# martinambrus/PitchExtractor

Measured on AMD Instinct MI355X. Metric: mel-frames/sec training throughput (JDCNet, 24 kHz, batch=256), higher is better.
Workload: dtype f32

## Files before the change

include/pitchextractor_hip.h:

```cpp
#ifndef PITCHEXTRACTOR_HIP_H
#define PITCHEXTRACTOR_HIP_H

#include <stddef.h>
#include <stdint.h>

#ifdef __cplusplus
extern "C" {
#endif

#define PE_OK 0
#define PE_E_ARG (-1)
#define PE_E_UNSUPPORTED (-2)
#define PE_E_WORKSPACE (-3)

enum pe_products {
  PE_PROD_NATIVE = 0,
  PE_PROD_X3 = 1,
  PE_PROD_H2 = 2,
  PE_PROD_BF16 = 3,
  PE_PROD_F16 = 4
};

int pe_abi_version(void);
int pe_device_count(void);
// ... 72 lines not shown
                         float eps, float momentum, float* running_mean, float* running_var, float* mean,
                         float* invstd, float* scale, float* shift, void* workspace, size_t workspace_bytes,
                         void* stream);
int pe_bn_eval_affine(const float* gamma, const float* beta, const float* running_mean,
                      const float* running_var, float eps, int C, float* scale, float* shift, void* stream);
int pe_bn_act_pool_fwd(int act16, const void* x, const float* scale, const float* shift, float slope, void* y, long rows,
                       int Fin, int C, int pool, long ldy, int coff, unsigned* amax_out, void* stream);
int pe_bn_act_pool_bwd(int act16, const void* x, const void* dy, const float* scale, const float* shift,
                       const float* mean, const float* invstd, float slope, void* dx, float* dgamma, float* dbeta,
                       long rows, int Fin, int C, int pool, long lddy, int coff, void* workspace,
                       size_t workspace_bytes, unsigned* amax_out, void* stream);
int pe_maxpool_fwd(int act16, const void* x, void* y, long rows, int Fin, int C, int pool, long ldy, int coff,
                   unsigned char* argmax_out, void* stream);
int pe_maxpool_bwd_add(int act16, const void* x, const unsigned char* argmax, const void* dy, void* dx, long rows,
                       int Fin, int C, int pool, long lddy, int coff, unsigned* amax_out, void* stream);
int pe_dropout_fwd(int act16, const void* x, long ldx, void* y, long ldy, const unsigned char* mask_in,
                   unsigned char* mask_out, long rows, int cols, float p, unsigned long long seed,
                   unsigned long long offset, void* stream);
int pe_nhwc_to_seq(int act16, const void* x, long ldx, int coff, float* seq, long rows, int C, void* stream);
int pe_seq_to_nhwc(int act16, const float* seq, void* x, long ldx, int coff, long rows, int C, int accumulate,
                   void* stream);
int pe_copy2d(int act16, const void* src, long lds, void* dst, long ldd, long rows, int cols, int accumulate,
              void* stream);

int pe_lstm_fwd(int ncells, const float* const* whh, float* const* gates, float* const* y,
                float* const* cbuf, const int* reverse, long ldy, int B, int T, int H, void* stream);
int pe_lstm_bwd(int ncells, const float* const* whh_t, float* const* gates, const float* const* cbuf,
                const float* const* dy, float* const* dcarry, const int* reverse, long lddy, int B, int T,
                int H, void* stream);
size_t pe_lstm_persistent_sync_bytes(int ncells, int B);
// ... 210 lines not shown
```

pitchextractor_amd/_lib.py:

```python
from __future__ import annotations

import ctypes as C
import os
from pathlib import Path

_PKG = Path(__file__).resolve().parent
LIB_PATH = Path(os.environ.get("PITCHEXTRACTOR_HIP_LIB", _PKG / "libpitchextractor_hip.so"))

_lib = None


class HipLibraryError(RuntimeError):
    pass


_p = C.c_void_p
_i = C.c_int
_l = C.c_long
_f = C.c_float
_d = C.c_double
_z = C.c_size_t
_u64 = C.c_ulonglong
_pp = C.POINTER(C.c_void_p)
_ip = C.POINTER(C.c_int)
# ... 28 lines not shown
    "pe_conv3x3_fwd_wf": (_i, [_i, _i, _p, _p, _p, _i, _i, _i, _i, _i, _i, _p, _p, _p, _p]),
    "pe_conv3x3_wgrad_workspace_bytes": (_z, [_i, _i, _i, _i, _i]),
    "pe_conv3x3_wgrad": (_i, [_i, _i, _p, _p, _p, _i, _i, _i, _i, _i, _p, _z, _p, _p, _p]),
    "pe_conv3x3_c1_stat_parts": (_i, [_i, _i, _i]),
    "pe_conv3x3_c1_fwd": (_i, [_i, _p, _l, _l, _l, _p, _p, _i, _i, _i, _p, _p]),
    "pe_conv3x3_c1_wgrad": (_i, [_i, _p, _l, _l, _l, _p, _p, _i, _i, _i, _p, _z, _p]),
    "pe_bn_workspace_bytes": (_z, [_i]),
    "pe_bn_train_stats": (_i, [_i, _p, _l, _i, _p, _p, _f, _f, _p, _p, _p, _p, _p, _p, _p, _z, _p]),
    "pe_conv3x3_wf_stat_parts": (_i, [_i, _i, _i]),
    "pe_bn_finalize_stats": (_i, [_p, _i, _l, _i, _p, _p, _f, _f, _p, _p, _p, _p, _p, _p, _p, _z, _p]),
    "pe_bn_eval_affine": (_i, [_p, _p, _p, _p, _f, _i, _p, _p, _p]),
    "pe_bn_act_pool_fwd": (_i, [_i, _p, _p, _p, _f, _p, _l, _i, _i, _i, _l, _i, _p, _p]),
    "pe_bn_act_pool_bwd": (_i, [_i, _p, _p, _p, _p, _p, _p, _f, _p, _p, _p, _l, _i, _i, _i, _l, _i, _p, _z, _p, _p]),
    "pe_maxpool_fwd": (_i, [_i, _p, _p, _l, _i, _i, _i, _l, _i, _p, _p]),
    "pe_maxpool_bwd_add": (_i, [_i, _p, _p, _p, _p, _l, _i, _i, _i, _l, _i, _p, _p]),
    "pe_dropout_fwd": (_i, [_i, _p, _l, _p, _l, _p, _p, _l, _i, _f, _u64, _u64, _p]),
    "pe_nhwc_to_seq": (_i, [_i, _p, _l, _i, _p, _l, _i, _p]),
    "pe_seq_to_nhwc": (_i, [_i, _p, _p, _l, _i, _l, _i, _i, _p]),
    "pe_copy2d": (_i, [_i, _p, _l, _p, _l, _l, _i, _i, _p]),
    "pe_lstm_fwd": (_i, [_i, _pp, _pp, _pp, _pp, _ip, _l, _i, _i, _i, _p]),
    "pe_lstm_bwd": (_i, [_i, _pp, _pp, _pp, _pp, _pp, _ip, _l, _i, _i, _i, _p]),
    "pe_lstm_persistent_sync_bytes": (_z, [_i, _i]),
    "pe_lstm_persistent_supported": (_i, [_i, _i, _i]),
    "pe_lstm_fwd_persistent": (_i, [_i, _i, _pp, _pp, _pp, _pp, _ip, _l, _i, _i, _i, _p, _p]),
    "pe_lstm_bwd_persistent_dbias_rows": (_i, [_i, _i, _i, _i, _l]),
    "pe_lstm_configure_stamps": (_i, [_i]),
    "pe_lstm_bwd_persistent": (_i, [_i, _i, _pp, _pp, _pp, _pp, _ip, _l, _i, _i, _i, _pp, _pp, _p, _p]),
    "pe_lstm_whh_grad_workspace_bytes": (_z, [_i, _i, _i]),
    "pe_lstm_whh_grad": (_i, [_i, _p, _p, _l, _p, _i, _i, _i, _i, _p, _z, _p, _p, _p]),
    "pe_colsum_workspace_bytes": (_z, [_i]),
# ... 140 lines not shown
```

pitchextractor_amd/csrc/elementwise.hip:

```cpp
#include <type_traits>
#include "forms.h"

namespace {
using namespace pe;

constexpr int kMaxPartials = 4096;

template <class F>
__device__ __forceinline__ void column_reduce2(F&& f, long n_pix, int C, double* partial ) {
  extern __shared__ __attribute__((aligned(16))) char smem_raw[];
  double* red = reinterpret_cast<double*>(smem_raw);
  const int quads = C >> 2;
  const int G = 256 / quads;
  const int q = threadIdx.x % quads, g = threadIdx.x / quads;
  double s1[4] = {0, 0, 0, 0}, s2[4] = {0, 0, 0, 0};
  if (g < G) {
    for (long p = (long)blockIdx.x * G + g; p < n_pix; p += (long)gridDim.x * G) {
      float4 a, b;
      f(p, q * 4, a, b);
      s1[0] += a.x; s1[1] += a.y; s1[2] += a.z; s1[3] += a.w;
      s2[0] += b.x; s2[1] += b.y; s2[2] += b.z; s2[3] += b.w;
    }
#pragma unroll
    for (int i = 0; i < 4; ++i) {
// ... 108 lines not shown
      const float4 v = ld4(xp + (long)j * C);
      float4 a;
      a.x = lrelu(fmaf(v.x, sc.x, sh.x), slope);
      a.y = lrelu(fmaf(v.y, sc.y, sh.y), slope);
      a.z = lrelu(fmaf(v.z, sc.z, sh.z), slope);
      a.w = lrelu(fmaf(v.w, sc.w, sh.w), slope);
      if (j == 0) m = a;
      else { m.x = fmaxf(m.x, a.x); m.y = fmaxf(m.y, a.y); m.z = fmaxf(m.z, a.z); m.w = fmaxf(m.w, a.w); }
    }
    st4(y + op * ldy + coff + q * 4, m);
    am = amax4(am, m);
  }
  amax_commit(am, amax);
}

__device__ __forceinline__ float dz_one(const float* __restrict__ xwin, long cstride, int j, int pool, float sc,
                                        float sh, float slope, float dyv) {
  float best = lrelu(fmaf(xwin[0], sc, sh), slope);
  int arg = 0;
  for (int k = 1; k < pool; ++k) {
    const float a = lrelu(fmaf(xwin[(long)k * cstride], sc, sh), slope);
    if (a > best) { best = a; arg = k; }
  }
  if (arg != j) return 0.f;
  const float z = fmaf(xwin[(long)j * cstride], sc, sh);
  return z > 0.f ? dyv : dyv * slope;
}

template <class TA>
struct BnBwdArgsT {
// ... 142 lines not shown
      [&](long item, int c, float4& s, float4& t) {
        BnWindow<POOL> w;
        bn_window<POOL, TA>(a, item, nwin, c, w, sc, sh);
        s = make_float4(0.f, 0.f, 0.f, 0.f);
        t = make_float4(0.f, 0.f, 0.f, 0.f);
#pragma unroll
        for (int j = 0; j < POOL; ++j) {
          s.x += w.dz[j].x; s.y += w.dz[j].y; s.z += w.dz[j].z; s.w += w.dz[j].w;
          t.x += w.dz[j].x * ((w.v[j].x - mu.x) * is.x); t.y += w.dz[j].y * ((w.v[j].y - mu.y) * is.y);
          t.z += w.dz[j].z * ((w.v[j].z - mu.z) * is.z); t.w += w.dz[j].w * ((w.v[j].w - mu.w) * is.w);
        }
      },
      n_items, a.C, partial);
}

template <int POOL, class TA>
__global__ __launch_bounds__(256) void bn_bwd_apply_win_kernel(const BnBwdArgsT<TA> a, long n_items, int nwin,
                                                               const float* __restrict__ c1,
                                                               const float* __restrict__ c2, TA* __restrict__ dx,
                                                               unsigned* __restrict__ amax) {
  const int quads = a.C >> 2;
  float am = 0.f;
  const int G = 256 / quads, c = (threadIdx.x % quads) * 4, g = threadIdx.x / quads;
  const float4 mu = *reinterpret_cast<const float4*>(a.mean + c), is = *reinterpret_cast<const float4*>(a.invstd + c);
  const float4 sc = *reinterpret_cast<const float4*>(a.scale + c), sh = *reinterpret_cast<const float4*>(a.shift + c);
  const float4 k1 = *reinterpret_cast<const float4*>(c1 + c), k2 = *reinterpret_cast<const float4*>(c2 + c);
  for (long item = (long)blockIdx.x * G + g; g < G && item < n_items; item += (long)gridDim.x * G) {
    BnWindow<POOL> w;
    bn_window<POOL, TA>(a, item, nwin, c, w, sc, sh);
#pragma unroll
    for (int j = 0; j < POOL; ++j) {
      if (j >= w.n) break;
      float4 o;
      o.x = sc.x * (w.dz[j].x - k1.x - (w.v[j].x - mu.x) * is.x * k2.x);
      o.y = sc.y * (w.dz[j].y - k1.y - (w.v[j].y - mu.y) * is.y * k2.y);
      o.z = sc.z * (w.dz[j].z - k1.z - (w.v[j].z - mu.z) * is.z * k2.z);
      o.w = sc.w * (w.dz[j].w - k1.w - (w.v[j].w - mu.w) * is.w * k2.w);
      st4(dx + (w.p0 + j) * a.C + c, o);
      am = amax4(am, o);
    }
  }
  amax_commit(am, amax);
}

template <class TA>
__global__ __launch_bounds__(256) void maxpool_fwd_kernel(const TA* __restrict__ x, TA* __restrict__ y,
                                                          long n_out_pix, int Fin, int C, int pool, long ldy,
                                                          int coff, unsigned char* __restrict__ arg) {
  const int quads = C >> 2, Fout = Fin / pool;
  const long total = n_out_pix * quads;
  for (long i = (long)blockIdx.x * 256 + threadIdx.x; i < total; i += (long)gridDim.x * 256) {
    const int q = (int)(i % quads);
    const long op = i / quads, row = op / Fout;
    const int fo = (int)(op % Fout);
// ... 298 lines not shown

extern "C" int pe_bn_act_pool_fwd(int act16, const void* x, const float* scale, const float* shift, float slope, void* y,
                                  long rows, int Fin, int C, int pool, long ldy, int coff, unsigned* amax_out,
                                  void* stream) {
  return with_act(act16, [&](auto a) {
    using TA = typename decltype(a)::TA;
    return bn_act_pool_fwd_impl(static_cast<const TA*>(x), scale, shift, slope, static_cast<TA*>(y), rows, Fin, C, pool,
                                ldy, coff, amax_out, stream);
  });
}

template <class TA>
static int bn_act_pool_bwd_impl(const TA* x, const TA* dy, const float* scale, const float* shift, const float* mean,
                                const float* invstd, float slope, TA* dx, float* dgamma, float* dbeta, long rows,
                                int Fin, int C, int pool, long lddy, int coff, void* workspace, size_t workspace_bytes,
                                unsigned* amax_out, void* stream) {
  if (!x || !dy || !scale || !shift || !mean || !invstd || !dx || !dgamma || !dbeta || rows <= 0) return PE_E_ARG;
  if (!bn_channels_ok(C) || (lddy & 3) || (coff & 3) || pool <= 0) return PE_E_UNSUPPORTED;
  const size_t need = pe_bn_workspace_bytes(C) + 2 * (size_t)C * sizeof(float);
  if (!workspace || workspace_bytes < need) return PE_E_WORKSPACE;
  hipStream_t st = pe_stream(stream);
  BnBwdArgsT<TA> a{x, dy, scale, shift, mean, invstd, slope, rows * Fin, Fin, C, pool, lddy, coff};
  double* partial = reinterpret_cast<double*>(workspace);
  float* c1 = reinterpret_cast<float*>(reinterpret_cast<char*>(workspace) + pe_bn_workspace_bytes(C));
  float* c2 = c1 + C;
  const int nwin = Fin / pool + (Fin % pool ? 1 : 0);
  const long n_items = rows * nwin;
  const bool win = pool == 1 || pool == 2 || pool == 4;
  if (!win && !std::is_same<TA, float>::value) return PE_E_UNSUPPORTED;
  const int grid = reduce_grid(win ? n_items : a.n_in_pix, C,
                               (!std::is_same<TA, float>::value && pool == 1) ? kMaxPartials : 1024);
  if (pool == 1)
    hipLaunchKernelGGL((bn_bwd_partial_win_kernel<1, TA>), dim3(grid), dim3(256), reduce_lds(C), st, a, n_items, nwin, partial);
  else if (pool == 2)
    hipLaunchKernelGGL((bn_bwd_partial_win_kernel<2, TA>), dim3(grid), dim3(256), reduce_lds(C), st, a, n_items, nwin, partial);
  else if (pool == 4)
    hipLaunchKernelGGL((bn_bwd_partial_win_kernel<4, TA>), dim3(grid), dim3(256), reduce_lds(C), st, a, n_items, nwin, partial);
  else if constexpr (std::is_same<TA, float>::value)
    hipLaunchKernelGGL(bn_bwd_partial_kernel, dim3(grid), dim3(256), reduce_lds(C), st, a, partial);
  PE_LAUNCH_CHECK();
  hipLaunchKernelGGL(bn_bwd_finalize_kernel, dim3(pe_cdiv(C, 4)), dim3(256), 0, st, partial, grid, a.n_in_pix, C,
                     dgamma, dbeta, c1, c2);
  PE_LAUNCH_CHECK();
  const int agrid = win ? ew_grid(pe_cdiv(n_items, 256 / (C / 4)) * 256L) : ew_grid(a.n_in_pix * (C / 4));
  if (pool == 1)
    hipLaunchKernelGGL((bn_bwd_apply_win_kernel<1, TA>), dim3(agrid), dim3(256), 0, st, a, n_items, nwin, c1, c2, dx,
                       amax_out);
  else if (pool == 2)
    hipLaunchKernelGGL((bn_bwd_apply_win_kernel<2, TA>), dim3(agrid), dim3(256), 0, st, a, n_items, nwin, c1, c2, dx,
                       amax_out);
  else if (pool == 4)
    hipLaunchKernelGGL((bn_bwd_apply_win_kernel<4, TA>), dim3(agrid), dim3(256), 0, st, a, n_items, nwin, c1, c2, dx,
                       amax_out);
  else if constexpr (std::is_same<TA, float>::value)
    hipLaunchKernelGGL(bn_bwd_apply_kernel, dim3(agrid), dim3(256), 0, st, a, c1, c2, dx, amax_out);
  PE_LAUNCH_CHECK();
  return PE_OK;
}

extern "C" int pe_bn_act_pool_bwd(int act16, const void* x, const void* dy, const float* scale, const float* shift,
                                  const float* mean, const float* invstd, float slope, void* dx, float* dgamma,
                                  float* dbeta, long rows, int Fin, int C, int pool, long lddy, int coff,
                                  void* workspace, size_t workspace_bytes, unsigned* amax_out, void* stream) {
  return with_act(act16, [&](auto a) {
    using TA = typename decltype(a)::TA;
    return bn_act_pool_bwd_impl(static_cast<const TA*>(x), static_cast<const TA*>(dy), scale, shift, mean, invstd, slope,
                                static_cast<TA*>(dx), dgamma, dbeta, rows, Fin, C, pool, lddy, coff, workspace,
                                workspace_bytes, amax_out, stream);
  });
}

template <class TA>
static int maxpool_fwd_impl(const TA* x, TA* y, long rows, int Fin, int C, int pool, long ldy, int coff,
                            unsigned char* argmax_out, void* stream) {
  if (!x || !y || rows <= 0 || Fin <= 0 || pool <= 0) return PE_E_ARG;
  if ((C & 3) || (ldy & 3) || (coff & 3) || (argmax_out && pool > 255)) return PE_E_UNSUPPORTED;
  const long n_out = rows * (Fin / pool);
  hipLaunchKernelGGL(maxpool_fwd_kernel<TA>, dim3(ew_grid(n_out * (C / 4))), dim3(256), 0, pe_stream(stream), x, y,
                     n_out, Fin, C, pool, ldy, coff, argmax_out);
  PE_LAUNCH_CHECK();
  return PE_OK;
}

extern "C" int pe_maxpool_fwd(int act16, const void* x, void* y, long rows, int Fin, int C, int pool, long ldy, int coff,
                              unsigned char* argmax_out, void* stream) {
  return with_act(act16, [&](auto a) {
// ... 124 lines not shown
```

pitchextractor_amd/model.py:

```python
from __future__ import annotations

import math
import os

import torch
from torch import nn

from . import ops

_ALIGN = 4


class _Conv(nn.Module):

    def __init__(self, cin, cout, k):
        super().__init__()
        self.weight = nn.Parameter(torch.empty(cout, cin, k, k))


class _BatchNorm(nn.Module):
    def __init__(self, c, eps=1e-5, momentum=0.1):
        super().__init__()
        self.eps, self.momentum = eps, momentum
        self.weight = nn.Parameter(torch.ones(c))
# ... 137 lines not shown
        st = ops.bn_train_stats(x, mod.weight, mod.bias, mod.running_mean, mod.running_var, mod.eps, mod.momentum,
                                partials=partials)
        mod.num_batches_tracked += 1
        return st
    return ops.bn_eval_affine(mod.weight, mod.bias, mod.running_mean, mod.running_var, mod.eps)


def _flat2(t):
    return t.view(-1, t.shape[-1])


def _no_amax(_param):
    return None


def _res_forward(blk: _ResBlock, x, pool, train, need_grad, slope, x_stats=None, wa=_no_amax):
    s = _Ctx()
    s.x = x
    s.bn_pre = _bn(blk.pre_conv[0], x, train, x_stats)
    s.am_p = ops.amax_word()
    s.p = ops.bn_act_pool_fwd(x, s.bn_pre, pool=pool, slope=slope, amax_out=s.am_p)
    out = ops.gemm_nt(_flat2(s.p), blk.conv1by1.weight.view(blk.cout, blk.cin), amax_a=s.am_p,
                      amax_b=wa(blk.conv1by1.weight))
    out = out.view(*s.p.shape[:3], blk.cout)
    wf0, s.wd0 = ops.conv3x3_repack(blk.conv[0].weight, True, need_grad, amax=wa(blk.conv[0].weight))
    s.c, c_stats = ops.conv3x3_fwd(s.p, wf0, bn_stats=train, amax=s.am_p)
    s.bn_mid = _bn(blk.conv[1], s.c, train, c_stats)
    s.am_a = ops.amax_word()
    s.a = ops.bn_act_pool_fwd(s.c, s.bn_mid, pool=1, slope=slope, amax_out=s.am_a)
    wf3, s.wd3 = ops.conv3x3_repack(blk.conv[3].weight, True, need_grad, amax=wa(blk.conv[3].weight))
    _, out_stats = ops.conv3x3_fwd(s.a, wf3, out=out, accumulate=True, bn_stats=train,
                                   amax=s.am_a)
    return out, s, out_stats


def _res_backward(blk: _ResBlock, s, d_out, pool, slope, grads, side, am_do=None, wa=_no_amax):
    if am_do is None:
        am_do = ops.amax_for(d_out)
    side.run(lambda: (ops.conv3x3_wgrad(s.a, d_out, grads[blk.conv[3].weight], amax_x=s.am_a, amax_dy=am_do),
                      ops.gemm_tn(_flat2(d_out), _flat2(s.p), out=grads[blk.conv1by1.weight].view(blk.cout, blk.cin),
                                  amax_a=am_do, amax_b=s.am_p)),
             d_out, am_do, on=OVERLAP_CONV_WGRAD)
    with ops.timer_tag("dgrad"):
        d_a = ops.conv3x3_fwd(d_out, s.wd3, amax=am_do)
    am_dc = ops.amax_word()
    d_c = ops.bn_act_pool_bwd(s.c, d_a, s.bn_mid, grads[blk.conv[1].weight], grads[blk.conv[1].bias], pool=1,
                              slope=slope, dx=d_a, amax_out=am_dc)
    side.run(lambda: ops.conv3x3_wgrad(s.p, d_c, grads[blk.conv[0].weight], amax_x=s.am_p, amax_dy=am_dc), d_c, am_dc,
             on=OVERLAP_CONV_WGRAD)
    with ops.timer_tag("dgrad"):
        d_p = ops.conv3x3_fwd(d_c, s.wd0, amax=am_dc)
    w1t = ops.transpose2d(blk.conv1by1.weight.view(blk.cout, blk.cin))
    ops.gemm_nt(_flat2(d_out), w1t, out=_flat2(d_p), accumulate=True, amax_a=am_do, amax_b=wa(blk.conv1by1.weight))
    am_dx = ops.amax_word()
    return ops.bn_act_pool_bwd(s.x, d_p, s.bn_pre, grads[blk.pre_conv[0].weight], grads[blk.pre_conv[0].bias],
                               pool=pool, slope=slope, amax_out=am_dx), am_dx


class _DropoutCfg:
    def __init__(self, seed=0):
        self.seed = int(seed)
        self.offset = 0
        self.inject = None

    def next_offset(self, n_quads):
        off = self.offset
        self.offset += int(n_quads)
        return off


def _dropout(cfg: _DropoutCfg, x2d, p, out2d=None):
# ... 89 lines not shown
        with torch.cuda.stream(side):
            fn()
        self.keep.append(keep)
        self.used = True

    def join(self):
        if self.used:
            torch.cuda.current_stream(self.dev).wait_stream(_side_stream(self.dev))
        self.keep.clear()
        self.used = False


OVERLAP_CONV_WGRAD = os.environ.get("PE_OVERLAP_CONV_WGRAD", "1") != "0"
OVERLAP_TF_WGRAD = os.environ.get("PE_OVERLAP_TF_WGRAD", "1") != "0"
LSTM_WGRAD_JOIN_EARLY = os.environ.get("PE_LSTM_WGRAD_JOIN", "early") == "early"


def _lstm_backward(models, saved, dys, grads, side, wa=_no_amax):
    m0 = models[0].model
    H, L, ND = m0.hidden_size, m0.num_layers, m0.num_dirs
    B, T = dys[0].shape[:2]
    dev = dys[0].device
    for layer in reversed(range(L)):
        lay = saved[layer]
        dys = [_dropout_bwd(_flat2(dys[mi]), lay.mask[mi][0], lay.mask[mi][1]).view(B, T, ND * H)
               for mi in range(len(models))]
        whh_t, dsl, dcs, rev = [], [], [], []
        for mi, sm in enumerate(models):
            for d in range(ND):
                _, w_hh, _, _ = sm.model.cell(layer, d)
# ... 367 lines not shown
        train = self.training
        slope = self.leaky_relu_slope
        self._refresh_weight_amax()
        s = _Ctx()
        x_btf = x[:, 0].float()
        B, T, F = x_btf.shape
        s.x_btf = x_btf
        cbk = self.conv_block
        s.y0, y0_stats = ops.conv3x3_c1_fwd(x_btf, cbk[0].weight, bn_stats=train)
        s.bn0 = _bn(cbk[1], s.y0, train, y0_stats)
        s.am_a0 = ops.amax_word()
        s.a0 = ops.bn_act_pool_fwd(s.y0, s.bn0, pool=1, slope=slope, amax_out=s.am_a0)
        wf, s.wd_cb = ops.conv3x3_repack(cbk[3].weight, True, need_grad, amax=self.weight_amax(cbk[3].weight))
        s.cb, st_cb = ops.conv3x3_fwd(s.a0, wf, bn_stats=train, amax=s.am_a0)
        wa = self.weight_amax
        s.rb1, s.r1, st1 = _res_forward(self.res_block1, s.cb, 2, train, need_grad, slope, st_cb, wa)
        s.rb2, s.r2, st2 = _res_forward(self.res_block2, s.rb1, 2, train, need_grad, slope, st1, wa)
        s.rb3, s.r3, st3 = _res_forward(self.res_block3, s.rb2, 2, train, need_grad, slope, st2, wa)

        Fp = s.rb3.shape[2] // 4
        if Fp != 2:
            raise ValueError("JDCNet geometry expects 80 mel bins (F/40 == 2)")
        s.bnp = _bn(self.pool_block[0], s.rb3, train, st3)
        pooled = ops.bn_act_pool_fwd(s.rb3, s.bnp, pool=4, slope=slope)
        s.concat = torch.empty((B, T, 2, 640), dtype=s.rb3.dtype, device=x.device)
        p_blk = self.block_dropout if train else 0.0
        cslice = s.concat.view(-1, 640)[:, 384:640]
        _, s.mask_pool = _dropout(self.dropout_cfg, _flat2(pooled), p_blk, out2d=cslice)
        seq_c = ops.nhwc_to_seq(s.concat, 256, coff=384)

        _, s.arg_cb = ops.maxpool_fwd(s.cb, 40, out=s.concat, coff=0, want_argmax=True)
        _, s.arg_rb1 = ops.maxpool_fwd(s.rb1, 20, out=s.concat, coff=64, want_argmax=True)
        _, s.arg_rb2 = ops.maxpool_fwd(s.rb2, 10, out=s.concat, coff=192, want_argmax=True)
        wdet = self.detector_conv[0].weight.view(256, 640)
        s.dconv = ops.gemm_nt(s.concat.view(-1, 640), wdet, amax_b=self.weight_amax(self.detector_conv[0].weight))
        s.dconv = s.dconv.view(B, T, 2, 256)
        s.bnd = _bn(self.detector_conv[1], s.dconv, train)
        dact = ops.bn_act_pool_fwd(s.dconv, s.bnd, pool=1, slope=slope)
        ddrop, s.mask_det = _dropout(self.dropout_cfg, _flat2(dact), p_blk)
        seq_d = ops.nhwc_to_seq(ddrop.view(B, T, 2, 256), 256)

        models = [self.sequence_classifier, self.sequence_detector]
        if models[0].model_type == "bilstm":
            (yc, yd), s.lstm = _lstm_forward(models, [seq_c, seq_d], train, need_grad, self.dropout_cfg, wa)
        else:
            yc, s.tf_c = _tf_forward(models[0], seq_c, train, need_grad, self.dropout_cfg)
            yd, s.tf_d = _tf_forward(models[1], seq_d, train, need_grad, self.dropout_cfg)
        s.yc, s.yd = yc, yd
# ... 58 lines not shown
        ops.seq_to_nhwc(dseq_c, d_concat, 256, coff=384, accumulate=True)
        d_pool = torch.empty((B, T, 2, 256), dtype=s.concat.dtype, device=dev)
        _dropout_bwd(d_concat.view(-1, 640)[:, 384:640], p_blk if s.mask_pool is not None else 0.0, s.mask_pool,
                     out2d=_flat2(d_pool))
        bnp = self.pool_block[0]
        am3 = ops.amax_word()
        d_rb3 = ops.bn_act_pool_bwd(s.rb3, d_pool, s.bnp, g[bnp.weight], g[bnp.bias], pool=4, slope=slope, amax_out=am3)

        cuts = self._dp_cuts if self._dp is not None else None

        def block_done(k):
            if cuts is not None:
                self._dp.reduce_range(cuts[k], cuts[k + 1], after=side.pending_stream())

        wa = self.weight_amax
        d_rb2, am2 = _res_backward(self.res_block3, s.r3, d_rb3, 2, slope, g, side, am3, wa)
        block_done(3)
        ops.maxpool_bwd_add(s.rb2, d_concat, d_rb2, 10, coff=192, amax_out=am2, argmax=s.arg_rb2)
        d_rb1, am1 = _res_backward(self.res_block2, s.r2, d_rb2, 2, slope, g, side, am2, wa)
        block_done(2)
        ops.maxpool_bwd_add(s.rb1, d_concat, d_rb1, 20, coff=64, amax_out=am1, argmax=s.arg_rb1)
        d_cb, am_dcb = _res_backward(self.res_block1, s.r1, d_rb1, 2, slope, g, side, am1, wa)
        block_done(1)
        ops.maxpool_bwd_add(s.cb, d_concat, d_cb, 40, coff=0, amax_out=am_dcb, argmax=s.arg_cb)

        cbk = self.conv_block
        side.run(lambda: ops.conv3x3_wgrad(s.a0, d_cb, g[cbk[3].weight], amax_x=s.am_a0, amax_dy=am_dcb), d_cb, am_dcb,
                 on=OVERLAP_CONV_WGRAD)
        with ops.timer_tag("dgrad"):
            d_a0 = ops.conv3x3_fwd(d_cb, s.wd_cb, amax=am_dcb)
        d_y0 = ops.bn_act_pool_bwd(s.y0, d_a0, s.bn0, g[cbk[1].weight], g[cbk[1].bias], pool=1, slope=slope, dx=d_a0)
        ops.conv3x3_c1_wgrad(s.x_btf, d_y0, g[cbk[0].weight])
        side.join()
        if self._dp is not None:
            self._dp.reduce_range(0, cuts[1] if cuts is not None else self._seq_offset())
```

pitchextractor_amd/ops.py:

```python
from __future__ import annotations

import ctypes as C

import os

import torch

from . import _lib

_WS: dict = {}


def _chk(cond, msg):
    if not cond:
        raise ValueError(msg)


def _f32c(t: torch.Tensor, name: str) -> torch.Tensor:
    _chk(t.is_cuda, f"{name}: expected a HIP device tensor (no CPU fallback)")
    _chk(t.dtype == torch.float32, f"{name}: expected float32")
    return t


def _dense(t: torch.Tensor, name: str) -> torch.Tensor:
# ... 447 lines not shown
    for t in (gamma, beta, running_mean, running_var):
        _chk(_dense(t, "bn tensor").numel() == Cc, "bn tensor size")
    _call("pe_bn_eval_affine", gamma.data_ptr(), beta.data_ptr(), running_mean.data_ptr(), running_var.data_ptr(),
          eps, Cc, st.scale.data_ptr(), st.shift.data_ptr(), _s())
    return st


def _slice_target(out, B, T, Fo, Cc, coff):
    _actd(out, "out")
    _chk(out.dim() == 4 and out.shape[:3] == (B, T, Fo), "output pixel grid mismatch")
    ld = out.shape[3]
    _chk(0 <= coff and coff + Cc <= ld, "channel slice out of range")
    return ld


def bn_act_pool_fwd(x, st: BnState, pool=1, slope=0.01, out=None, coff=0, amax_out=None):
    x = _actd(x, "x")
    B, T, F, Cc = x.shape
    Fo = F // pool
    if out is None:
        out = torch.empty((B, T, Fo, Cc), dtype=x.dtype, device=x.device)
    ld = _slice_target(out, B, T, Fo, Cc, coff)
    _call("pe_bn_act_pool_fwd", x.data_ptr(), st.scale.data_ptr(), st.shift.data_ptr(), slope, out.data_ptr(),
          B * T, F, Cc, pool, ld, coff, _lib.ptr(amax_out), _s(), act16=_act16(x, out))
    return out


def bn_act_pool_bwd(x, dy, st: BnState, dgamma, dbeta, pool=1, slope=0.01, coff=0, dx=None, amax_out=None):
    x = _actd(x, "x")
    B, T, F, Cc = x.shape
    ld = _slice_target(dy, B, T, F // pool, Cc, coff)
    if dx is None:
        dx = torch.empty_like(x)
    _chk(_actd(dx, "dx").shape == x.shape, "dx shape")
    _chk(_dense(dgamma, "dgamma").numel() == Cc and _dense(dbeta, "dbeta").numel() == Cc, "dgamma/dbeta size")
    lib = _lib.load()
    ws = workspace(lib.pe_bn_workspace_bytes(Cc) + 8 * Cc, x.device)
    _call("pe_bn_act_pool_bwd", x.data_ptr(), dy.data_ptr(), st.scale.data_ptr(), st.shift.data_ptr(),
          st.mean.data_ptr(), st.invstd.data_ptr(), slope, dx.data_ptr(), dgamma.data_ptr(), dbeta.data_ptr(),
          B * T, F, Cc, pool, ld, coff, ws.data_ptr(), ws.numel(), _lib.ptr(amax_out), _s(), act16=_act16(x, dy, dx))
    return dx


def maxpool_fwd(x, pool, out=None, coff=0, want_argmax=False):
    x = _actd(x, "x")
    B, T, F, Cc = x.shape
    Fo = F // pool
    if out is None:
        out = torch.empty((B, T, Fo, Cc), dtype=x.dtype, device=x.device)
    ld = _slice_target(out, B, T, Fo, Cc, coff)
    arg = torch.empty((B, T, Fo, Cc), dtype=torch.uint8, device=x.device) if want_argmax else None
    _call("pe_maxpool_fwd", x.data_ptr(), out.data_ptr(), B * T, F, Cc, pool, ld, coff, _lib.ptr(arg), _s(),
          act16=_act16(x, out))
    return (out, arg) if want_argmax else out

# ... 593 lines not shown
```

Before: 642,100.

## Fold detector-concat maxpool taps into BN-act-pool forward and backward kernels

Adds fused kernels that compute the wide frequency max-pool tap (with argmax) into the concat buffer while running the BN+LeakyReLU+pool pass, and that add the tap gradient inside the BN backward apply kernel. This removes three separate maxpool forward and three maxpool backward-add launches, along with their re-reads of the residual block activations. The forward kernel uses a shared-memory segment reduction whose width is chosen at launch. It adds complexity and per-element argmax comparisons, and is gated by an environment flag that defaults on.

```diff
diff --git a/include/pitchextractor_hip.h b/include/pitchextractor_hip.h
--- a/include/pitchextractor_hip.h
+++ b/include/pitchextractor_hip.h
@@ -110,6 +110,15 @@
                    unsigned char* argmax_out, void* stream);
 int pe_maxpool_bwd_add(int act16, const void* x, const unsigned char* argmax, const void* dy, void* dx, long rows,
                        int Fin, int C, int pool, long lddy, int coff, unsigned* amax_out, void* stream);
+int pe_bn_act_pool_tap_supported(long rows, int Fin, int C, int pool, int tap_pool, int with_arg);
+int pe_bn_act_pool_tap_fwd(int act16, const void* x, const float* scale, const float* shift, float slope, void* y,
+                           long rows, int Fin, int C, int pool, long ldy, int coff, unsigned* amax_out, void* tap_y,
+                           long tap_ldy, int tap_coff, int tap_pool, unsigned char* tap_arg, void* stream);
+int pe_bn_act_pool_tap_bwd(int act16, const void* x, const void* dy, const float* scale, const float* shift,
+                           const float* mean, const float* invstd, float slope, void* dx, float* dgamma, float* dbeta,
+                           long rows, int Fin, int C, int pool, long lddy, int coff, void* workspace,
+                           size_t workspace_bytes, unsigned* amax_out, const void* tap_dy, long tap_lddy, int tap_coff,
+                           int tap_pool, const unsigned char* tap_arg, void* stream);
 int pe_dropout_fwd(int act16, const void* x, long ldx, void* y, long ldy, const unsigned char* mask_in,
                    unsigned char* mask_out, long rows, int cols, float p, unsigned long long seed,
                    unsigned long long offset, void* stream);
diff --git a/pitchextractor_amd/_lib.py b/pitchextractor_amd/_lib.py
--- a/pitchextractor_amd/_lib.py
+++ b/pitchextractor_amd/_lib.py
@@ -66,6 +66,10 @@
     "pe_bn_act_pool_bwd": (_i, [_i, _p, _p, _p, _p, _p, _p, _f, _p, _p, _p, _l, _i, _i, _i, _l, _i, _p, _z, _p, _p]),
     "pe_maxpool_fwd": (_i, [_i, _p, _p, _l, _i, _i, _i, _l, _i, _p, _p]),
     "pe_maxpool_bwd_add": (_i, [_i, _p, _p, _p, _p, _l, _i, _i, _i, _l, _i, _p, _p]),
+    "pe_bn_act_pool_tap_supported": (_i, [_l, _i, _i, _i, _i, _i]),
+    "pe_bn_act_pool_tap_fwd": (_i, [_i, _p, _p, _p, _f, _p, _l, _i, _i, _i, _l, _i, _p, _p, _l, _i, _i, _p, _p]),
+    "pe_bn_act_pool_tap_bwd": (_i, [_i, _p, _p, _p, _p, _p, _p, _f, _p, _p, _p, _l, _i, _i, _i, _l, _i, _p, _z, _p,
+                                    _p, _l, _i, _i, _p, _p]),
     "pe_dropout_fwd": (_i, [_i, _p, _l, _p, _l, _p, _p, _l, _i, _f, _u64, _u64, _p]),
     "pe_nhwc_to_seq": (_i, [_i, _p, _l, _i, _p, _l, _i, _p]),
     "pe_seq_to_nhwc": (_i, [_i, _p, _p, _l, _i, _l, _i, _i, _p]),
diff --git a/pitchextractor_amd/csrc/elementwise.hip b/pitchextractor_amd/csrc/elementwise.hip
--- a/pitchextractor_amd/csrc/elementwise.hip
+++ b/pitchextractor_amd/csrc/elementwise.hip
@@ -146,6 +146,84 @@
   amax_commit(am, amax);
 }
 
+template <int POOL, class TA>
+__global__ __launch_bounds__(256) void bn_act_pool_tap_fwd_kernel(const TA* __restrict__ x,
+                                                                  const float* __restrict__ scale,
+                                                                  const float* __restrict__ shift, float slope,
+                                                                  TA* __restrict__ y, long n_tap, int C, int nbw, int S,
+                                                                  long ldy, int coff, unsigned* __restrict__ amax,
+                                                                  TA* __restrict__ tap_y, long tap_ldy, int tap_coff,
+                                                                  unsigned char* __restrict__ tap_arg) {
+  __shared__ float4 tap_val[2][256];
+  __shared__ uchar4 tap_pos[2][256];
+  const int quads = C >> 2;
+  const int G = 256 / quads, q = threadIdx.x % quads, g = threadIdx.x / quads;
+  const int TW = G / S, segw = nbw / S;
+  const int wl = g / S, seg = g - wl * S;
+  const bool lane_on = g < TW * S;
+  const float4 sc = *reinterpret_cast<const float4*>(scale + q * 4), sh = *reinterpret_cast<const float4*>(shift + q * 4);
+  const long n_trips = (n_tap + TW - 1) / TW;
+  float am = 0.f;
+  int buf = 0;
+  for (long trip = blockIdx.x; trip < n_trips; trip += gridDim.x, buf ^= 1) {
+    const long tw = trip * TW + wl;
+    const bool on = lane_on && tw < n_tap;
+    const float ninf = -__builtin_inff();
+    float4 tm = make_float4(ninf, ninf, ninf, ninf);
+    int a0 = seg * segw * POOL, a1 = a0, a2 = a0, a3 = a0;
+    if (on) {
+      const long op0 = tw * nbw + (long)seg * segw;
+      const TA* xp = x + (op0 * POOL * C + q * 4);
+      TA* yp = y + (op0 * ldy + coff + q * 4);
+      int pos = seg * segw * POOL;
+      bool first = seg == 0;
+      for (int i = 0; i < segw; ++i, xp += (long)POOL * C, yp += ldy) {
+        float4 v[POOL];
+#pragma unroll
+        for (int j = 0; j < POOL; ++j) v[j] = ld4(xp + (long)j * C);
+        float4 m;
+#pragma unroll
+        for (int j = 0; j < POOL; ++j, ++pos) {
+          float4 a;
+          a.x = lrelu(fmaf(v[j].x, sc.x, sh.x), slope);
+          a.y = lrelu(fmaf(v[j].y, sc.y, sh.y), slope);
+          a.z = lrelu(fmaf(v[j].z, sc.z, sh.z), slope);
+          a.w = lrelu(fmaf(v[j].w, sc.w, sh.w), slope);
+          if (j == 0) m = a;
+          else { m.x = fmaxf(m.x, a.x); m.y = fmaxf(m.y, a.y); m.z = fmaxf(m.z, a.z); m.w = fmaxf(m.w, a.w); }
+          if (first || v[j].x > tm.x) { tm.x = v[j].x; a0 = pos; }
+          if (first || v[j].y > tm.y) { tm.y = v[j].y; a1 = pos; }
+          if (first || v[j].z > tm.z) { tm.z = v[j].z; a2 = pos; }
+          if (first || v[j].w > tm.w) { tm.w = v[j].w; a3 = pos; }
+          first = false;
+        }
+        st4(yp, m);
+        am = amax4(am, m);
+      }
+      if (S > 1) {
+        tap_val[buf][threadIdx.x] = tm;
+        tap_pos[buf][threadIdx.x] = make_uchar4((unsigned char)a0, (unsigned char)a1, (unsigned char)a2, (unsigned char)a3);
+      }
+    }
+    if (S > 1) __syncthreads();
+    if (on && seg == 0) {
+      for (int k = 1; k < S; ++k) {
+        const float4 o = tap_val[buf][threadIdx.x + k * quads];
+        const uchar4 p = tap_pos[buf][threadIdx.x + k * quads];
+        if (o.x > tm.x) { tm.x = o.x; a0 = p.x; }
+        if (o.y > tm.y) { tm.y = o.y; a1 = p.y; }
+        if (o.z > tm.z) { tm.z = o.z; a2 = p.z; }
+        if (o.w > tm.w) { tm.w = o.w; a3 = p.w; }
+      }
+      st4(tap_y + tw * tap_ldy + tap_coff + q * 4, tm);
+      if (tap_arg != nullptr)
+        *reinterpret_cast<uchar4*>(tap_arg + tw * C + q * 4) = make_uchar4((unsigned char)a0, (unsigned char)a1,
+                                                                           (unsigned char)a2, (unsigned char)a3);
+    }
+  }
+  amax_commit(am, amax);
+}
+
 __device__ __forceinline__ float dz_one(const float* __restrict__ xwin, long cstride, int j, int pool, float sc,
                                         float sh, float slope, float dyv) {
   float best = lrelu(fmaf(xwin[0], sc, sh), slope);
@@ -318,6 +396,24 @@
       n_items, a.C, partial);
 }
 
+template <class TA>
+struct BnTapGrad {
+  const TA* dy;
+  const unsigned char* arg;
+  long lddy;
+  int coff;
+  unsigned nbw;
+};
+
+__device__ __forceinline__ float round_act(const float*, float v) { return v; }
+__device__ __forceinline__ float round_act(const act16_t*, float v) {
+  return __uint_as_float(pack_bf16_rne(v, 0.f) << 16);
+}
+__device__ __forceinline__ float add_unfused(float a, float b) {
+#pragma clang fp contract(off)
+  return a + b;
+}
+
 template <int POOL, class TA>
 __global__ __launch_bounds__(256) void bn_bwd_apply_win_kernel(const BnBwdArgsT<TA> a, long n_items, int nwin,
                                                                const float* __restrict__ c1,
@@ -342,6 +438,44 @@
       o.w = sc.w * (w.dz[j].w - k1.w - (w.v[j].w - mu.w) * is.w * k2.w);
       st4(dx + (w.p0 + j) * a.C + c, o);
       am = amax4(am, o);
+    }
+  }
+  amax_commit(am, amax);
+}
+
+template <int POOL, class TA>
+__global__ __launch_bounds__(256) void bn_bwd_apply_win_tap_kernel(const BnBwdArgsT<TA> a, long n_items, int nwin,
+                                                                   const float* __restrict__ c1,
+                                                                   const float* __restrict__ c2, TA* __restrict__ dx,
+                                                                   unsigned* __restrict__ amax, const BnTapGrad<TA> t) {
+  const int quads = a.C >> 2;
+  float am = 0.f;
+  const int G = 256 / quads, c = (threadIdx.x % quads) * 4, g = threadIdx.x / quads;
+  const float4 mu = *reinterpret_cast<const float4*>(a.mean + c), is = *reinterpret_cast<const float4*>(a.invstd + c);
+  const float4 sc = *reinterpret_cast<const float4*>(a.scale + c), sh = *reinterpret_cast<const float4*>(a.shift + c);
+  const float4 k1 = *reinterpret_cast<const float4*>(c1 + c), k2 = *reinterpret_cast<const float4*>(c2 + c);
+  for (long item = (long)blockIdx.x * G + g; g < G && item < n_items; item += (long)gridDim.x * G) {
+    BnWindow<POOL> w;
+    bn_window<POOL, TA>(a, item, nwin, c, w, sc, sh);
+    const unsigned tw = (unsigned)item / t.nbw;
+    const int pos0 = (int)((unsigned)item - tw * t.nbw) * POOL;
+    const uchar4 ar = *reinterpret_cast<const uchar4*>(t.arg + (long)tw * a.C + c);
+    const float4 tg = ld4(t.dy + (long)tw * t.lddy + t.coff + c);
+#pragma unroll
+    for (int j = 0; j < POOL; ++j) {
+      if (j >= w.n) break;
+      float4 o;
+      o.x = sc.x * (w.dz[j].x - k1.x - (w.v[j].x - mu.x) * is.x * k2.x);
+      o.y = sc.y * (w.dz[j].y - k1.y - (w.v[j].y - mu.y) * is.y * k2.y);
+      o.z = sc.z * (w.dz[j].z - k1.z - (w.v[j].z - mu.z) * is.z * k2.z);
+      o.w = sc.w * (w.dz[j].w - k1.w - (w.v[j].w - mu.w) * is.w * k2.w);
+      am = amax4(am, o);
+      const int pj = pos0 + j;
+      if (ar.x == pj) { o.x = add_unfused(round_act(dx, o.x), tg.x); am = fmaxf(am, fabsf(o.x)); }
+      if (ar.y == pj) { o.y = add_unfused(round_act(dx, o.y), tg.y); am = fmaxf(am, fabsf(o.y)); }
+      if (ar.z == pj) { o.z = add_unfused(round_act(dx, o.z), tg.z); am = fmaxf(am, fabsf(o.z)); }
+      if (ar.w == pj) { o.w = add_unfused(round_act(dx, o.w), tg.w); am = fmaxf(am, fabsf(o.w)); }
+      st4(dx + (w.p0 + j) * a.C + c, o);
     }
   }
   amax_commit(am, amax);
@@ -670,7 +804,7 @@
 static int bn_act_pool_bwd_impl(const TA* x, const TA* dy, const float* scale, const float* shift, const float* mean,
                                 const float* invstd, float slope, TA* dx, float* dgamma, float* dbeta, long rows,
                                 int Fin, int C, int pool, long lddy, int coff, void* workspace, size_t workspace_bytes,
-                                unsigned* amax_out, void* stream) {
+                                unsigned* amax_out, void* stream, const BnTapGrad<TA>* tap = nullptr) {
   if (!x || !dy || !scale || !shift || !mean || !invstd || !dx || !dgamma || !dbeta || rows <= 0) return PE_E_ARG;
   if (!bn_channels_ok(C) || (lddy & 3) || (coff & 3) || pool <= 0) return PE_E_UNSUPPORTED;
   const size_t need = pe_bn_workspace_bytes(C) + 2 * (size_t)C * sizeof(float);
@@ -699,7 +833,17 @@
                      dgamma, dbeta, c1, c2);
   PE_LAUNCH_CHECK();
   const int agrid = win ? ew_grid(pe_cdiv(n_items, 256 / (C / 4)) * 256L) : ew_grid(a.n_in_pix * (C / 4));
-  if (pool == 1)
+  if (tap != nullptr) {
+    if (pool == 1)
+      hipLaunchKernelGGL((bn_bwd_apply_win_tap_kernel<1, TA>), dim3(agrid), dim3(256), 0, st, a, n_items, nwin, c1, c2,
+                         dx, amax_out, *tap);
+    else if (pool == 2)
+      hipLaunchKernelGGL((bn_bwd_apply_win_tap_kernel<2, TA>), dim3(agrid), dim3(256), 0, st, a, n_items, nwin, c1, c2,
+                         dx, amax_out, *tap);
+    else
+      hipLaunchKernelGGL((bn_bwd_apply_win_tap_kernel<4, TA>), dim3(agrid), dim3(256), 0, st, a, n_items, nwin, c1, c2,
+                         dx, amax_out, *tap);
+  } else if (pool == 1)
     hipLaunchKernelGGL((bn_bwd_apply_win_kernel<1, TA>), dim3(agrid), dim3(256), 0, st, a, n_items, nwin, c1, c2, dx,
                        amax_out);
   else if (pool == 2)
@@ -726,6 +870,79 @@
   });
 }
 
+static bool tap_geometry_ok(long rows, int Fin, int C, int pool, int tap_pool, bool with_arg) {
+  if (!bn_channels_ok(C) || rows <= 0 || Fin <= 0) return false;
+  if (pool != 1 && pool != 2 && pool != 4) return false;
+  if (tap_pool <= 0 || tap_pool % pool != 0 || Fin % tap_pool != 0) return false;
+  if (with_arg && tap_pool > 255) return false;
+  return rows * (long)Fin < (1L << 31);
+}
+
+extern "C" int pe_bn_act_pool_tap_supported(long rows, int Fin, int C, int pool, int tap_pool, int with_arg) {
+  return tap_geometry_ok(rows, Fin, C, pool, tap_pool, with_arg != 0) ? 1 : 0;
+}
+
+template <class TA>
+static int bn_act_pool_tap_fwd_impl(const TA* x, const float* scale, const float* shift, float slope, TA* y, long rows,
+                                    int Fin, int C, int pool, long ldy, int coff, unsigned* amax_out, TA* tap_y,
+                                    long tap_ldy, int tap_coff, int tap_pool, unsigned char* tap_arg, void* stream) {
+  if (!x || !scale || !shift || !y || !tap_y || rows <= 0 || Fin <= 0 || pool <= 0) return PE_E_ARG;
+  if ((ldy & 3) || (coff & 3) || (tap_ldy & 3) || (tap_coff & 3) ||
+      !tap_geometry_ok(rows, Fin, C, pool, tap_pool, tap_arg != nullptr))
+    return PE_E_UNSUPPORTED;
+  const int G = 256 / (C / 4), nbw = tap_pool / pool;
+  int S = 1, used = 0;
+  for (int s = 1; s <= G && s <= nbw; ++s) {
+    if (nbw % s) continue;
+    const int u = (G / s) * s;
+    if (u >= used) { used = u; S = s; }
+  }
+  const long n_tap = rows * (Fin / tap_pool), n_trips = pe_cdiv(n_tap, (long)(G / S));
+  const dim3 grid(ew_grid(n_trips * 256L));
+  hipStream_t st = pe_stream(stream);
+  if (pool == 1)
+    hipLaunchKernelGGL((bn_act_pool_tap_fwd_kernel<1, TA>), grid, dim3(256), 0, st, x, scale, shift, slope, y, n_tap, C,
+                       nbw, S, ldy, coff, amax_out, tap_y, tap_ldy, tap_coff, tap_arg);
+  else if (pool == 2)
+    hipLaunchKernelGGL((bn_act_pool_tap_fwd_kernel<2, TA>), grid, dim3(256), 0, st, x, scale, shift, slope, y, n_tap, C,
+                       nbw, S, ldy, coff, amax_out, tap_y, tap_ldy, tap_coff, tap_arg);
+  else
+    hipLaunchKernelGGL((bn_act_pool_tap_fwd_kernel<4, TA>), grid, dim3(256), 0, st, x, scale, shift, slope, y, n_tap, C,
+                       nbw, S, ldy, coff, amax_out, tap_y, tap_ldy, tap_coff, tap_arg);
+  PE_LAUNCH_CHECK();
+  return PE_OK;
+}
+
+extern "C" int pe_bn_act_pool_tap_fwd(int act16, const void* x, const float* scale, const float* shift, float slope,
+                                      void* y, long rows, int Fin, int C, int pool, long ldy, int coff,
+                                      unsigned* amax_out, void* tap_y, long tap_ldy, int tap_coff, int tap_pool,
+                                      unsigned char* tap_arg, void* stream) {
+  return with_act(act16, [&](auto a) {
+    using TA = typename decltype(a)::TA;
+    return bn_act_pool_tap_fwd_impl(static_cast<const TA*>(x), scale, shift, slope, static_cast<TA*>(y), rows, Fin, C,
+                                    pool, ldy, coff, amax_out, static_cast<TA*>(tap_y), tap_ldy, tap_coff, tap_pool,
+                                    tap_arg, stream);
+  });
+}
+
+extern "C" int pe_bn_act_pool_tap_bwd(int act16, const void* x, const void* dy, const float* scale, const float* shift,
+                                      const float* mean, const float* invstd, float slope, void* dx, float* dgamma,
+                                      float* dbeta, long rows, int Fin, int C, int pool, long lddy, int coff,
+                                      void* workspace, size_t workspace_bytes, unsigned* amax_out, const void* tap_dy,
+                                      long tap_lddy, int tap_coff, int tap_pool, const unsigned char* tap_arg,
+                                      void* stream) {
+  return with_act(act16, [&](auto a) {
+    using TA = typename decltype(a)::TA;
+    if (!tap_dy || !tap_arg) return (int)PE_E_ARG;
+    if ((tap_lddy & 3) || (tap_coff & 3) || !tap_geometry_ok(rows, Fin, C, pool, tap_pool, true))
+      return (int)PE_E_UNSUPPORTED;
+    const BnTapGrad<TA> tap{static_cast<const TA*>(tap_dy), tap_arg, tap_lddy, tap_coff, (unsigned)(tap_pool / pool)};
+    return bn_act_pool_bwd_impl(static_cast<const TA*>(x), static_cast<const TA*>(dy), scale, shift, mean, invstd, slope,
+                                static_cast<TA*>(dx), dgamma, dbeta, rows, Fin, C, pool, lddy, coff, workspace,
+                                workspace_bytes, amax_out, stream, &tap);
+  });
+}
+
 template <class TA>
 static int maxpool_fwd_impl(const TA* x, TA* y, long rows, int Fin, int C, int pool, long ldy, int coff,
                             unsigned char* argmax_out, void* stream) {
diff --git a/pitchextractor_amd/model.py b/pitchextractor_amd/model.py
--- a/pitchextractor_amd/model.py
+++ b/pitchextractor_amd/model.py
@@ -175,12 +175,12 @@
     return None
 
 
-def _res_forward(blk: _ResBlock, x, pool, train, need_grad, slope, x_stats=None, wa=_no_amax):
+def _res_forward(blk: _ResBlock, x, pool, train, need_grad, slope, x_stats=None, wa=_no_amax, tap=None):
     s = _Ctx()
     s.x = x
     s.bn_pre = _bn(blk.pre_conv[0], x, train, x_stats)
     s.am_p = ops.amax_word()
-    s.p = ops.bn_act_pool_fwd(x, s.bn_pre, pool=pool, slope=slope, amax_out=s.am_p)
+    s.p = ops.bn_act_pool_fwd(x, s.bn_pre, pool=pool, slope=slope, amax_out=s.am_p, tap=tap)
     out = ops.gemm_nt(_flat2(s.p), blk.conv1by1.weight.view(blk.cout, blk.cin), amax_a=s.am_p,
                       amax_b=wa(blk.conv1by1.weight))
     out = out.view(*s.p.shape[:3], blk.cout)
@@ -195,7 +195,7 @@
     return out, s, out_stats
 
 
-def _res_backward(blk: _ResBlock, s, d_out, pool, slope, grads, side, am_do=None, wa=_no_amax):
+def _res_backward(blk: _ResBlock, s, d_out, pool, slope, grads, side, am_do=None, wa=_no_amax, tap=None):
     if am_do is None:
         am_do = ops.amax_for(d_out)
     side.run(lambda: (ops.conv3x3_wgrad(s.a, d_out, grads[blk.conv[3].weight], amax_x=s.am_a, amax_dy=am_do),
@@ -215,7 +215,7 @@
     ops.gemm_nt(_flat2(d_out), w1t, out=_flat2(d_p), accumulate=True, amax_a=am_do, amax_b=wa(blk.conv1by1.weight))
     am_dx = ops.amax_word()
     return ops.bn_act_pool_bwd(s.x, d_p, s.bn_pre, grads[blk.pre_conv[0].weight], grads[blk.pre_conv[0].bias],
-                               pool=pool, slope=slope, amax_out=am_dx), am_dx
+                               pool=pool, slope=slope, amax_out=am_dx, tap=tap), am_dx
 
 
 class _DropoutCfg:
@@ -335,6 +335,7 @@
 OVERLAP_CONV_WGRAD = os.environ.get("PE_OVERLAP_CONV_WGRAD", "1") != "0"
 OVERLAP_TF_WGRAD = os.environ.get("PE_OVERLAP_TF_WGRAD", "1") != "0"
 LSTM_WGRAD_JOIN_EARLY = os.environ.get("PE_LSTM_WGRAD_JOIN", "early") == "early"
+FOLD_TAPS = os.environ.get("PE_FOLD_TAPS", "1") != "0"
 
 
 def _lstm_backward(models, saved, dys, grads, side, wa=_no_amax):
@@ -732,24 +733,31 @@
         wf, s.wd_cb = ops.conv3x3_repack(cbk[3].weight, True, need_grad, amax=self.weight_amax(cbk[3].weight))
         s.cb, st_cb = ops.conv3x3_fwd(s.a0, wf, bn_stats=train, amax=s.am_a0)
         wa = self.weight_amax
-        s.rb1, s.r1, st1 = _res_forward(self.res_block1, s.cb, 2, train, need_grad, slope, st_cb, wa)
-        s.rb2, s.r2, st2 = _res_forward(self.res_block2, s.rb1, 2, train, need_grad, slope, st1, wa)
-        s.rb3, s.r3, st3 = _res_forward(self.res_block3, s.rb2, 2, train, need_grad, slope, st2, wa)
+        s.taps = None
+        if FOLD_TAPS:
+            s.concat = torch.empty((B, T, 2, 640), dtype=s.cb.dtype, device=x.device)
+            s.taps = [ops.Tap(s.concat, tp, coff, want_argmax=need_grad) for tp, coff in ((40, 0), (20, 64), (10, 192))]
+        t_cb, t_rb1, t_rb2 = s.taps or (None, None, None)
+        s.rb1, s.r1, st1 = _res_forward(self.res_block1, s.cb, 2, train, need_grad, slope, st_cb, wa, t_cb)
+        s.rb2, s.r2, st2 = _res_forward(self.res_block2, s.rb1, 2, train, need_grad, slope, st1, wa, t_rb1)
+        s.rb3, s.r3, st3 = _res_forward(self.res_block3, s.rb2, 2, train, need_grad, slope, st2, wa, t_rb2)
 
         Fp = s.rb3.shape[2] // 4
         if Fp != 2:
             raise ValueError("JDCNet geometry expects 80 mel bins (F/40 == 2)")
         s.bnp = _bn(self.pool_block[0], s.rb3, train, st3)
         pooled = ops.bn_act_pool_fwd(s.rb3, s.bnp, pool=4, slope=slope)
-        s.concat = torch.empty((B, T, 2, 640), dtype=s.rb3.dtype, device=x.device)
+        if s.taps is None:
+            s.concat = torch.empty((B, T, 2, 640), dtype=s.rb3.dtype, device=x.device)
         p_blk = self.block_dropout if train else 0.0
         cslice = s.concat.view(-1, 640)[:, 384:640]
         _, s.mask_pool = _dropout(self.dropout_cfg, _flat2(pooled), p_blk, out2d=cslice)
         seq_c = ops.nhwc_to_seq(s.concat, 256, coff=384)
 
-        _, s.arg_cb = ops.maxpool_fwd(s.cb, 40, out=s.concat, coff=0, want_argmax=True)
-        _, s.arg_rb1 = ops.maxpool_fwd(s.rb1, 20, out=s.concat, coff=64, want_argmax=True)
-        _, s.arg_rb2 = ops.maxpool_fwd(s.rb2, 10, out=s.concat, coff=192, want_argmax=True)
+        if s.taps is None:
+            _, s.arg_cb = ops.maxpool_fwd(s.cb, 40, out=s.concat, coff=0, want_argmax=True)
+            _, s.arg_rb1 = ops.maxpool_fwd(s.rb1, 20, out=s.concat, coff=64, want_argmax=True)
+            _, s.arg_rb2 = ops.maxpool_fwd(s.rb2, 10, out=s.concat, coff=192, want_argmax=True)
         wdet = self.detector_conv[0].weight.view(256, 640)
         s.dconv = ops.gemm_nt(s.concat.view(-1, 640), wdet, amax_b=self.weight_amax(self.detector_conv[0].weight))
         s.dconv = s.dconv.view(B, T, 2, 256)
@@ -838,15 +846,21 @@
                 self._dp.reduce_range(cuts[k], cuts[k + 1], after=side.pending_stream())
 
         wa = self.weight_amax
-        d_rb2, am2 = _res_backward(self.res_block3, s.r3, d_rb3, 2, slope, g, side, am3, wa)
+        t_cb, t_rb1, t_rb2 = s.taps or (None, None, None)
+        for t in s.taps or ():
+            t.grad = d_concat
+        d_rb2, am2 = _res_backward(self.res_block3, s.r3, d_rb3, 2, slope, g, side, am3, wa, t_rb2)
         block_done(3)
-        ops.maxpool_bwd_add(s.rb2, d_concat, d_rb2, 10, coff=192, amax_out=am2, argmax=s.arg_rb2)
-        d_rb1, am1 = _res_backward(self.res_block2, s.r2, d_rb2, 2, slope, g, side, am2, wa)
+        if s.taps is None:
+            ops.maxpool_bwd_add(s.rb2, d_concat, d_rb2, 10, coff=192, amax_out=am2, argmax=s.arg_rb2)
+        d_rb1, am1 = _res_backward(self.res_block2, s.r2, d_rb2, 2, slope, g, side, am2, wa, t_rb1)
         block_done(2)
-        ops.maxpool_bwd_add(s.rb1, d_concat, d_rb1, 20, coff=64, amax_out=am1, argmax=s.arg_rb1)
-        d_cb, am_dcb = _res_backward(self.res_block1, s.r1, d_rb1, 2, slope, g, side, am1, wa)
+        if s.taps is None:
+            ops.maxpool_bwd_add(s.rb1, d_concat, d_rb1, 20, coff=64, amax_out=am1, argmax=s.arg_rb1)
+        d_cb, am_dcb = _res_backward(self.res_block1, s.r1, d_rb1, 2, slope, g, side, am1, wa, t_cb)
         block_done(1)
-        ops.maxpool_bwd_add(s.cb, d_concat, d_cb, 40, coff=0, amax_out=am_dcb, argmax=s.arg_cb)
+        if s.taps is None:
+            ops.maxpool_bwd_add(s.cb, d_concat, d_cb, 40, coff=0, amax_out=am_dcb, argmax=s.arg_cb)
 
         cbk = self.conv_block
         side.run(lambda: ops.conv3x3_wgrad(s.a0, d_cb, g[cbk[3].weight], amax_x=s.am_a0, amax_dy=am_dcb), d_cb, am_dcb,
diff --git a/pitchextractor_amd/ops.py b/pitchextractor_amd/ops.py
--- a/pitchextractor_amd/ops.py
+++ b/pitchextractor_amd/ops.py
@@ -485,19 +485,46 @@
     return ld
 
 
-def bn_act_pool_fwd(x, st: BnState, pool=1, slope=0.01, out=None, coff=0, amax_out=None):
+class Tap:
+
+    def __init__(self, out, pool, coff, want_argmax=False):
+        self.out, self.pool, self.coff, self.want_argmax = out, int(pool), int(coff), bool(want_argmax)
+        self.argmax = None
+        self.grad = None
+
+
+def _tap_folded(x, pool, tap: Tap, with_arg) -> bool:
+    B, T, F, Cc = x.shape
+    return bool(_lib.load().pe_bn_act_pool_tap_supported(B * T, F, Cc, pool, tap.pool, int(with_arg)))
+
+
+def bn_act_pool_fwd(x, st: BnState, pool=1, slope=0.01, out=None, coff=0, amax_out=None, tap: Tap | None = None):
     x = _actd(x, "x")
     B, T, F, Cc = x.shape
     Fo = F // pool
     if out is None:
         out = torch.empty((B, T, Fo, Cc), dtype=x.dtype, device=x.device)
     ld = _slice_target(out, B, T, Fo, Cc, coff)
+    if tap is not None and _tap_folded(x, pool, tap, tap.want_argmax):
+        Ft = F // tap.pool
+        tld = _slice_target(tap.out, B, T, Ft, Cc, tap.coff)
+        tap.argmax = torch.empty((B, T, Ft, Cc), dtype=torch.uint8, device=x.device) if tap.want_argmax else None
+        _call("pe_bn_act_pool_tap_fwd", x.data_ptr(), st.scale.data_ptr(), st.shift.data_ptr(), slope, out.data_ptr(),
+              B * T, F, Cc, pool, ld, coff, _lib.ptr(amax_out), tap.out.data_ptr(), tld, tap.coff, tap.pool,
+              _lib.ptr(tap.argmax), _s(), act16=_act16(x, out, tap.out))
+        return out
     _call("pe_bn_act_pool_fwd", x.data_ptr(), st.scale.data_ptr(), st.shift.data_ptr(), slope, out.data_ptr(),
           B * T, F, Cc, pool, ld, coff, _lib.ptr(amax_out), _s(), act16=_act16(x, out))
-    return out
-
-
-def bn_act_pool_bwd(x, dy, st: BnState, dgamma, dbeta, pool=1, slope=0.01, coff=0, dx=None, amax_out=None):
+    if tap is not None:
+        if tap.want_argmax:
+            _, tap.argmax = maxpool_fwd(x, tap.pool, out=tap.out, coff=tap.coff, want_argmax=True)
+        else:
+            maxpool_fwd(x, tap.pool, out=tap.out, coff=tap.coff)
+    return out
+
+
+def bn_act_pool_bwd(x, dy, st: BnState, dgamma, dbeta, pool=1, slope=0.01, coff=0, dx=None, amax_out=None,
+                    tap: Tap | None = None):
     x = _actd(x, "x")
     B, T, F, Cc = x.shape
     ld = _slice_target(dy, B, T, F // pool, Cc, coff)
@@ -507,9 +534,21 @@
     _chk(_dense(dgamma, "dgamma").numel() == Cc and _dense(dbeta, "dbeta").numel() == Cc, "dgamma/dbeta size")
     lib = _lib.load()
     ws = workspace(lib.pe_bn_workspace_bytes(Cc) + 8 * Cc, x.device)
+    if tap is not None and tap.argmax is not None and _tap_folded(x, pool, tap, True):
+        Ft = F // tap.pool
+        _chk(tap.argmax.is_cuda and tap.argmax.dtype == torch.uint8 and tap.argmax.is_contiguous()
+             and tap.argmax.shape == (B, T, Ft, Cc), "bn_act_pool_bwd: tap argmax shape")
+        tld = _slice_target(tap.grad, B, T, Ft, Cc, tap.coff)
+        _call("pe_bn_act_pool_tap_bwd", x.data_ptr(), dy.data_ptr(), st.scale.data_ptr(), st.shift.data_ptr(),
+              st.mean.data_ptr(), st.invstd.data_ptr(), slope, dx.data_ptr(), dgamma.data_ptr(), dbeta.data_ptr(),
+              B * T, F, Cc, pool, ld, coff, ws.data_ptr(), ws.numel(), _lib.ptr(amax_out), tap.grad.data_ptr(), tld,
+              tap.coff, tap.pool, tap.argmax.data_ptr(), _s(), act16=_act16(x, dy, dx, tap.grad))
+        return dx
     _call("pe_bn_act_pool_bwd", x.data_ptr(), dy.data_ptr(), st.scale.data_ptr(), st.shift.data_ptr(),
           st.mean.data_ptr(), st.invstd.data_ptr(), slope, dx.data_ptr(), dgamma.data_ptr(), dbeta.data_ptr(),
           B * T, F, Cc, pool, ld, coff, ws.data_ptr(), ws.numel(), _lib.ptr(amax_out), _s(), act16=_act16(x, dy, dx))
+    if tap is not None:
+        maxpool_bwd_add(x, tap.grad, dx, tap.pool, coff=tap.coff, amax_out=amax_out, argmax=tap.argmax)
     return dx
 
 
```

Result: faster. 651,300, median of 6 (+1.4%).
